# Cyan4973/FiniteStateEntropy

Measured on AMD Instinct MI355X. Metric: MB/s encode+decode per GPU on 32KB probagen blocks; bit-exact vs CPU ref, higher is better.
Workload: dtype u8; 1 GPU; probagen Proba14, 100000 x 32KB blocks per GPU, FSE encode+decode (one-shot calls at the reference's default limits: tableLog 11, decode maxLog 12), bit-exact check; blocks_per_gpu=100000, block_bytes=32768, codec=fse, parity=fse: roundtrip-all-blocks

## Files before the change

finitestateentropy_amd/csrc/fse_tables.hip:

```cpp
#include "internal.h"

#include "wave_glue.h"
#include "ncount_reader.h"
#include "fse_wave_build.h"

template <u32 MAXC>
DEV void fse_wave_build_ctable(const WaveBuildLds& w, const int nn[4], u32 maxSV, u32 tl, u32* img, u32 lane)
{
    u16* const cumAll = w.cumP;
    *(uint2*)(w.nrm + 4 * lane) = make_uint2(((u32)nn[0] & 0xFFFFu) | ((u32)nn[1] << 16), ((u32)nn[2] & 0xFFFFu) | ((u32)nn[3] << 16));
    __syncthreads();
    const u32 ts = 1u << tl;
    u16* const stateTable = (u16*)(img + 1);
    u32* const tt = img + 1 + (ts >> 1);
    {
        u32 eff[4], laneSum = 0;
#pragma unroll
        for (int i = 0; i < 4; ++i) { eff[i] = nn[i] == -1 ? 1u : (u32)nn[i]; laneSum += eff[i]; }
        u32 total;
        u32 run = wb_scan_excl(laneSum, lane, &total);
#pragma unroll
        for (int i = 0; i < 4; ++i) {
            const u32 s = 4 * lane + i;
            cumAll[s] = (u16)run;
            if (s <= maxSV) {
                if (nn[i] == 0) { tt[2 * s] = 0; tt[2 * s + 1] = ((tl + 1) << 16) - ts; }
                else if (nn[i] == -1 || nn[i] == 1) { tt[2 * s] = run - 1u; tt[2 * s + 1] = (tl << 16) - ts; }
                else {
                    const u32 maxBitsOut = tl - hibit32((u32)nn[i] - 1);
                    tt[2 * s] = run - (u32)nn[i];
                    tt[2 * s + 1] = (maxBitsOut << 16) - ((u32)nn[i] << maxBitsOut);
                }
            }
            run += eff[i];
        }
        if (lane == 0) img[0] = tl | (maxSV << 16);
    }
    __syncthreads();
    wave_spread_rank<MAXC>(w, maxSV, tl, lane, [&](u32 s) { return (u32)cumAll[s]; },
                     [&](u32 u, u32 s, u32 r, u32 first) { (void)s; stateTable[first + r] = (u16)(ts + u); });
}

template <u32 MAXC>
__global__ __launch_bounds__(64) void k_fse_cprep(FseCPrepArgs a, u32 capTs)
{
    extern __shared__ __attribute__((aligned(16))) u8 wbLds[];
    const size_t b = blockIdx.x;
    const u32 lane = threadIdx.x;
    const size_t n = view_size(a.src, b);
    FseMeta m; m.state = 0; m.hdrSize = 0; m.tableLog = 0; m.maxSV = 0; m.pace = 0;
    const size_t top = a.histResults[b];
    size_t result = 0; bool go = false;
    if (n <= 1) result = 0;
    else if (is_err(top)) result = top;
    else if (top == n) result = 1;
    else if (top == 1 || top < (n >> 7)) result = 0;
    else go = true;
    const WaveBuildLds w = wave_build_carve(wbLds, capTs, true);
    u32* const hdrImg = w.cnt;
    u32 maxSV = 0, tl = 0;
    int nn[4] = { 0, 0, 0, 0 };
    if (go) {
        maxSV = a.maxSVs[b];
        tl = wg_optimal_tablelog(a.tableLogReq, n, maxSV, 2);
        if ((1u << tl) > 64u * MAXC || (1u << tl) > capTs) { result = FERR(tableLog_tooLarge); go = false; }
    }
    if (go) {
        const uint4 cv = ((const uint4*)(a.counts + b * 256))[lane];
        const u32 c[4] = { cv.x, cv.y, cv.z, cv.w };
        for (u32 i = lane; i < 136; i += 64) hdrImg[i] = 0;
        const size_t e = wg_normalize<64>(nn, c, (u64)n, maxSV, tl, lane);
        if (is_err(e)) { result = e; go = false; }
    }
    __syncthreads();
    if (go) {
        const size_t h = wg_write_ncount<64>(hdrImg, a.dstCapacity, nn, maxSV, tl, lane);
        if (is_err(h)) { result = h; go = false; }
        else m.hdrSize = (u32)h;
    }
    __syncthreads();
    if (!go) { if (lane == 0) { a.meta[b] = m; a.results[b] = result; } return; }
    {   u8* const dst = a.dst + b * a.dstStride;
        const u8* const hb = (const u8*)hdrImg;
        for (u32 i = lane; i < m.hdrSize; i += 64) dst[i] = hb[i];
    }
    int top1 = nn[0] > nn[1] ? nn[0] : nn[1]; top1 = nn[2] > top1 ? nn[2] : top1; top1 = nn[3] > top1 ? nn[3] : top1;
    top1 = wave_max_i32(top1);
    m.state = ((u32)top1 * 64u > (63u << tl) || n < FSE_ENC_WAVE_MIN) ? FSE_ENC_LANE : FSE_ENC_PAR;
    {
        u32 present = (nn[0] != 0) + (nn[1] != 0) + (nn[2] != 0) + (nn[3] != 0);
        present = wg_sum<64>(present);
        const u32 mix = (1u << tl) / (present ? present : 1u);
        m.pace = mix < 64u ? 0u : mix < 128u ? 1u : mix < 256u ? 2u : 3u;
    }
    m.tableLog = tl; m.maxSV = maxSV;
    if (lane == 0) a.meta[b] = m;
    fse_wave_build_ctable<MAXC>(w, nn, maxSV, tl, a.ctables + b * a.ctStrideU32, lane);
}

__global__ __launch_bounds__(64) void k_fse_dparse(FseDPrepArgs a)
{
    __shared__ __attribute__((aligned(16))) u32 stage[NCS_WORDS];
    const size_t b0 = (size_t)blockIdx.x * 64, b = b0 + threadIdx.x;
    const u32 lane = threadIdx.x;
    const bool have = b < a.nBlocks;
    const u8* const in = have ? view_ptr(a.csrc, b) : nullptr;
    const size_t cSize = have ? view_size(a.csrc, b) : 0;
    bool done = false;
    if (have && a.rawRle) { const size_t orig = a.origSizes ? a.origSizes[b] : a.uniformOrig; done = cSize == orig || cSize == 1; }
    const u32 staged = ncount_stage(stage, in, cSize, lane, have && !done);
    {   uint4* const rows = (uint4*)(a.norms + b0 * 256);
        const u32 nRows = a.nBlocks - b0 < 64 ? (u32)(a.nBlocks - b0) : 64u;
        for (u32 i = lane; i < nRows * 32u; i += 64) rows[i] = make_uint4(0, 0, 0, 0);
    }
    __syncthreads();
    int cls = -1;
    if (have) {
        FseMeta m; m.state = 0; m.hdrSize = 0; m.tableLog = 0; m.maxSV = 0; m.pace = 0; m.pace = 0;
        size_t result = 0;
        if (!done) do {
            u32 tl = 0, maxSV = 255;
            s16* const norm = a.norms + b * 256;
            const size_t h = ncount_read_staged(norm, &maxSV, &tl, stage + lane, staged, in, cSize);
            if (is_err(h)) { result = h; break; }
            if (tl > a.maxLog) { result = FERR(tableLog_tooLarge); break; }
            cls = FSE_DCLS_REV11;
            if (tl > FSE_DEC_FAST_MAXLOG) {
                int top = 0;
                for (u32 i = 0; i <= maxSV >> 3; ++i) {
                    const uint4 v = ((const uint4*)norm)[i];
                    const u32 q[4] = { v.x, v.y, v.z, v.w };
#pragma unroll
                    for (int k = 0; k < 4; ++k) { const int lo = (s16)(q[k] & 0xFFFFu), hi = (s16)(q[k] >> 16); top = lo > top ? lo : top; top = hi > top ? hi : top; }
                }
                cls = 2 * top > (1 << tl) ? FSE_DCLS_PLAIN : FSE_DCLS_REV12;
            }
            m.state = 1u | ((u32)cls << 2); m.hdrSize = (u32)h; m.tableLog = tl; m.maxSV = maxSV;
        } while (0);
        a.meta[b] = m;
        if (m.state == 0 && !done) a.results[b] = result;
    }
    if (cls >= 0) { const size_t bin = view_size(a.csrc, b) >> FSE_DBIN_LOG; cls = cls * FSE_DBINS + (int)(bin < FSE_DBINS - 1 ? bin : FSE_DBINS - 1); }
    const unsigned long long below = (1ull << lane) - 1ull;
    unsigned long long todo = __ballot(cls >= 0);
    while (todo) {
        const int leader = __builtin_ctzll(todo);
        const int c = __shfl(cls, leader, WAVE);
        const unsigned long long mask = __ballot(cls == c);
        u32 base = 0;
        if ((int)lane == leader) {
            base = atomicAdd(&a.counts[c], (u32)__builtin_popcountll(mask));
            atomicAdd(&a.counts[FSE_DCLS_COUNT + c / FSE_DBINS], (u32)__builtin_popcountll(mask));
        }
        base = (u32)__shfl((int)base, leader, WAVE);
        if (cls == c) a.lists[(size_t)c * a.nBlocks + base + (u32)__builtin_popcountll(mask & below)] = (u32)b;
        todo &= ~mask;
    }
}

template <u32 MAXC>
__global__ __launch_bounds__(64) void k_fse_dbuild(FseDPrepArgs a, u32 capTs, int firstList, int nLists, u32 ldsCapTs)
{
    extern __shared__ __attribute__((aligned(16))) u8 wbLds[];
    {   u32 total = 0;
        for (int k = firstList / (int)FSE_DBINS; k < (firstList + nLists) / (int)FSE_DBINS; ++k) total += a.counts[FSE_DCLS_COUNT + k];
        if (blockIdx.x >= total) return;
    }
    constexpr int MAXL = 2 * FSE_DBINS;
    static_assert(FSE_DBINS % 4 == 0, "the list lengths are read as 16-byte vectors");
    uint4 cv[MAXL / 4];
#pragma unroll
    for (int i = 0; i < MAXL / 4; ++i) cv[i] = 4 * i < nLists ? ((const uint4*)(a.counts + firstList))[i] : make_uint4(0, 0, 0, 0);
    u32 idx = blockIdx.x;
    int c = firstList + nLists;
    {   u32 before = 0; bool found = false;
#pragma unroll
        for (int i = 0; i < MAXL; ++i) {
            const uint4 v = cv[i >> 2];
            const u32 n = (i & 3) == 0 ? v.x : (i & 3) == 1 ? v.y : (i & 3) == 2 ? v.z : v.w;
            const bool here = !found & (i < nLists) & (idx < before + n);
            c = here ? firstList + i : c; idx = here ? idx - before : idx;
            found |= here;
            before += n;
        }
    }
    if (c == firstList + nLists) return;
    const size_t b = a.lists[(size_t)c * a.nBlocks + idx];
    const u32 lane = threadIdx.x;
    const FseMeta m = a.meta[b];
    if (m.state == 0) return;
    const u32 tl = m.tableLog, ts = 1u << tl;
    if (ts > ldsCapTs || ts > 64u * MAXC) {
        if (lane == 0) { a.meta[b].state = 0; a.results[b] = FERR(tableLog_tooLarge); }
        return;
    }
    const WaveBuildLds w = wave_build_carve(wbLds, ldsCapTs, false);
    *(uint2*)(w.nrm + 4 * lane) = *(const uint2*)(a.norms + b * 256 + 4 * lane);
    __syncthreads();
    const bool rev = ((m.state >> 2) & 3u) != FSE_DCLS_PLAIN;
    u16* const A = a.atab + b * capTs;
    u8* const S = a.symtab + b * capTs;
    const bool fast = wave_spread_rank<MAXC>(w, m.maxSV, tl, lane, [&](u32 s) { return (u32)(int)w.nrm[s]; }, [&](u32 u, u32 s, u32 r, u32 nrm) {
        const int n = (int)nrm;
        const u32 next = (n > 0 ? (u32)n : 1u) + r;
        const u32 nb = tl - hibit32(next);
        const u32 ns = (next << nb) - ts;
        const u32 x = rev ? __brev(u) >> (32u - tl) : u;
        A[x] = rev ? (u16)(nb | ((__brev(ns) >> (32u - tl)) << 5)) : (u16)((ns & 0xFFFu) | (nb << 12));
        S[x] = (u8)s;
    });
    if (lane == 0) a.meta[b].state = m.state | (fast ? 2u : 0u);
}

__global__ __launch_bounds__(256) void k_fse_export_dtable(FseDPrepArgs a, u32 capTs, u32* dtables, size_t dtStrideU32)
{
    const size_t b = blockIdx.x;
    const FseMeta m = a.meta[b];
    if (m.state == 0) return;
    const u32 tl = m.tableLog, ts = 1u << tl;
    const bool rev = ((m.state >> 2) & 3u) != FSE_DCLS_PLAIN;
    const u16* const A = a.atab + b * capTs;
    const u8* const S = a.symtab + b * capTs;
    u32* const dt = dtables + b * dtStrideU32;
    if (threadIdx.x == 0) dt[0] = tl | ((m.state & 2u) ? 1u << 16 : 0u);
    for (u32 x = threadIdx.x; x < ts; x += blockDim.x) {
        const u32 i = rev ? __brev(x) >> (32u - tl) : x;
        const u32 c = A[i];
        const u32 nb = rev ? (c & 31u) : (c >> 12);
        const u32 ns = rev ? __brev(c >> 5) >> (32u - tl) : (c & 0xFFFu);
        dt[1 + x] = ns | ((u32)S[i] << 16) | (nb << 24);
    }
}
hipError_t launch_fse_export_dtables(const FseDPrepArgs& a, u32* dtables, size_t dtStrideU32, hipStream_t s)
{
    if (a.nBlocks == 0) return hipSuccess;
    hipLaunchKernelGGL(k_fse_export_dtable, dim3((unsigned)a.nBlocks), dim3(256), 0, s, a, 1u << a.maxLog, dtables, dtStrideU32);
    return hipGetLastError();
}

DEV size_t fse_norm_load_checked(int nn[4], const s16* nb, u32 maxSV, u32 tl, u32 maxTl, u32 lane)
{
    if (maxSV > 255u) return FERR(maxSymbolValue_tooLarge);
    if (tl > maxTl) return FERR(tableLog_tooLarge);
    if (tl == 0 || tl == 1 || tl == 3) return FERR(GENERIC);
    u32 cells = 0; bool bad = false;
#pragma unroll
    for (int i = 0; i < 4; ++i) {
        nn[i] = 4 * lane + i <= maxSV ? (int)nb[4 * lane + i] : 0;
        bad |= nn[i] < -1;
        cells += nn[i] == -1 ? 1u : nn[i] > 0 ? (u32)nn[i] : 0u;
    }
    cells = wg_sum<64>(cells);
    return (wg_any<64>(bad, lane) || cells != (1u << tl)) ? FERR(GENERIC) : 0;
}
template <u32 MAXC>
__global__ __launch_bounds__(64) void k_fse_ctable_from_norm(const s16* norms, size_t normStride, const u32* maxSVs, u32 tl, u32* ctables, size_t ctStrideU32,
                                                            size_t* results, u32 capTs)
{
    extern __shared__ __attribute__((aligned(16))) u8 wbLds[];
    const size_t b = blockIdx.x;
    const u32 lane = threadIdx.x;
    const u32 maxSV = maxSVs[b];
    int nn[4] = { 0, 0, 0, 0 };
    static_assert(MAXC == 32 || MAXC == 64, "64 * MAXC cells = a table of tableLog 11 or 12");
    const size_t r = fse_norm_load_checked(nn, norms + b * normStride, maxSV, tl, MAXC == 32 ? 11u : FSE_MAX_TL, lane);
    if (lane == 0) results[b] = r;
    if (is_err(r)) return;
    fse_wave_build_ctable<MAXC>(wave_build_carve(wbLds, capTs, true), nn, maxSV, tl, ctables + b * ctStrideU32, lane);
}
hipError_t launch_fse_ctable_from_norm(const s16* norms, size_t normStride, const u32* maxSVs, u32 tl, u32* ctables, size_t ctStrideU32, size_t* results,
                                       size_t nBlocks, hipStream_t s)
{
    if (nBlocks == 0) return hipSuccess;
    const u32 capTs = 1u << (tl >= 1 && tl <= FSE_MAX_TL ? tl : FSE_MAX_TL);
    if (wb_small(capTs))
        hipLaunchKernelGGL(k_fse_ctable_from_norm<32>, dim3((unsigned)nBlocks), dim3(64), wave_build_lds_bytes(capTs, true), s, norms, normStride, maxSVs, tl, ctables,
                           ctStrideU32, results, capTs);
    else
        hipLaunchKernelGGL(k_fse_ctable_from_norm<64>, dim3((unsigned)nBlocks), dim3(64), wave_build_lds_bytes(capTs, true), s, norms, normStride, maxSVs, tl, ctables,
                           ctStrideU32, results, capTs);
    return hipGetLastError();
}

static void launch_fse_dbuild_lists(const FseDPrepArgs& a, u32 capTs, int firstList, int nLists, u32 ldsCapTs, hipStream_t s)
{
    if (wb_small(ldsCapTs))
        hipLaunchKernelGGL(k_fse_dbuild<32>, dim3((unsigned)a.nBlocks), dim3(64), wave_build_lds_bytes(ldsCapTs, false), s, a, capTs, firstList, nLists, ldsCapTs);
    else
        hipLaunchKernelGGL(k_fse_dbuild<64>, dim3((unsigned)a.nBlocks), dim3(64), wave_build_lds_bytes(ldsCapTs, false), s, a, capTs, firstList, nLists, ldsCapTs);
}
static void launch_fse_dbuilds(const FseDPrepArgs& a, hipStream_t s)
{
    const u32 capTs = 1u << a.maxLog;
    const u32 capA = a.maxLog < FSE_DEC_FAST_MAXLOG ? capTs : (1u << FSE_DEC_FAST_MAXLOG);
    launch_fse_dbuild_lists(a, capTs, (int)FSE_DCLS_REV11 * FSE_DBINS, (int)FSE_DBINS, capA, s);
    if (a.maxLog > FSE_DEC_FAST_MAXLOG) launch_fse_dbuild_lists(a, capTs, (int)FSE_DCLS_REV12 * FSE_DBINS, 2 * (int)FSE_DBINS, capTs, s);
}

__global__ __launch_bounds__(64) void k_fse_dmeta_from_norm(FseDPrepArgs a, const s16* norms, size_t normStride, const u32* maxSVs, u32 tl)
{
    const size_t b = blockIdx.x;
    const u32 lane = threadIdx.x;
    const u32 maxSV = maxSVs[b];
    int nn[4] = { 0, 0, 0, 0 };
    const size_t r = fse_norm_load_checked(nn, norms + b * normStride, maxSV, tl, a.maxLog, lane);
    FseMeta m; m.state = 0; m.hdrSize = 0; m.tableLog = tl; m.maxSV = maxSV; m.pace = 0;
    if (!is_err(r)) {
        *(uint2*)(a.norms + b * 256 + 4 * lane) = make_uint2(((u32)nn[0] & 0xFFFFu) | ((u32)nn[1] << 16), ((u32)nn[2] & 0xFFFFu) | ((u32)nn[3] << 16));
        int top = nn[0] > nn[1] ? nn[0] : nn[1]; top = nn[2] > top ? nn[2] : top; top = nn[3] > top ? nn[3] : top;
        top = wave_max_i32(top);
        const u32 cls = tl <= FSE_DEC_FAST_MAXLOG ? (u32)FSE_DCLS_REV11 : 2 * top > (1 << tl) ? (u32)FSE_DCLS_PLAIN : (u32)FSE_DCLS_REV12;
        m.state = 1u | (cls << 2);
        if (lane == 0) {
            const u32 at = atomicAdd(&a.counts[cls * FSE_DBINS], 1u);
            atomicAdd(&a.counts[FSE_DCLS_COUNT + cls], 1u);
            a.lists[(size_t)cls * FSE_DBINS * a.nBlocks + at] = (u32)b;
        }
    }
    if (lane == 0) { a.meta[b] = m; if (is_err(r)) a.results[b] = r; }
}
hipError_t launch_fse_dprep_from_norm(const FseDPrepArgs& a, const s16* norms, size_t normStride, const u32* maxSVs, u32 tl, hipStream_t s)
{
    if (a.nBlocks == 0) return hipSuccess;
    hipError_t e = launch_zero_u32(a.counts, FSE_DCLS_COUNT + FSE_DCLS_KINDS, s);
    if (e != hipSuccess) return e;
    hipLaunchKernelGGL(k_fse_dmeta_from_norm, dim3((unsigned)a.nBlocks), dim3(64), 0, s, a, norms, normStride, maxSVs, tl);
    launch_fse_dbuilds(a, s);
    return hipGetLastError();
}

#ifdef FSE_WB_TIMING
extern "C" __attribute__((visibility("default"))) int FSEHIP_debug_wbTiming(unsigned long long* host) { return (int)hipMemcpyFromSymbol(host, HIP_SYMBOL(g_wbTiming), sizeof(g_wbTiming)); }
#endif
__global__ __launch_bounds__(64) void k_fse_glue_normalize(s16* norms, size_t normStride, u32 tlReq, const u32* counts, size_t countStride,
                                                          const size_t* totals, const u32* maxSVs, size_t* results)
{
    const size_t b = blockIdx.x;
    const u32 lane = threadIdx.x;
    const u32 maxSV = maxSVs[b] > 255u ? 255u : maxSVs[b];
    const u32* const cb = counts + b * countStride;
    u32 c[4];
#pragma unroll
    for (int i = 0; i < 4; ++i) c[i] = 4 * lane + i <= maxSV ? cb[4 * lane + i] : 0u;
    int nn[4] = { 0, 0, 0, 0 };
    const u32 tl = tlReq ? tlReq : FSE_DEF_TL;
    const u64 total = (u64)totals[b];
    size_t r = total ? wg_normalize<64>(nn, c, total, maxSV, tl, lane) : FERR(GENERIC);
    if (!is_err(r)) r = tl;
    s16* const nb = norms + b * normStride;
#pragma unroll
    for (int i = 0; i < 4; ++i) if (4 * lane + i <= maxSV && !is_err(r)) nb[4 * lane + i] = (s16)nn[i];
    if (lane == 0) results[b] = r;
}

__global__ __launch_bounds__(64) void k_fse_glue_write_ncount(u8* headers, size_t headerStride, size_t headerCapacity, const s16* norms, size_t normStride,
                                                             const u32* maxSVs, u32 tl, size_t* results)
{
    __shared__ u32 img[136];
    const size_t b = blockIdx.x;
    const u32 lane = threadIdx.x;
    const u32 maxSV = maxSVs[b];
    size_t r;
    if (tl > FSE_MAX_TL) r = FERR(tableLog_tooLarge);
    else if (tl < FSE_MIN_TL || maxSV > 255u) r = FERR(GENERIC);
    else {
        const s16* const nb = norms + b * normStride;
        int nn[4];
#pragma unroll
        for (int i = 0; i < 4; ++i) nn[i] = 4 * lane + i <= maxSV ? (int)nb[4 * lane + i] : 0;
        for (u32 i = lane; i < 136; i += 64) img[i] = 0;
        __syncthreads();
        r = wg_write_ncount<64>(img, headerCapacity, nn, maxSV, tl, lane);
        __syncthreads();
        if (!is_err(r)) {
            u8* const dst = headers + b * headerStride;
            const u8* const hb = (const u8*)img;
            for (u32 i = lane; i < (u32)r; i += 64) dst[i] = hb[i];
        }
    }
    if (lane == 0) results[b] = r;
}

__global__ __launch_bounds__(64) void k_fse_glue_read_ncount(s16* norms, size_t normStride, u32* maxSVs, u32* tableLogs, BlockView headers, size_t nBlocks, size_t* results)
{
    const size_t b = (size_t)blockIdx.x * 64 + threadIdx.x;
    if (b >= nBlocks) return;
    u32 maxSV = maxSVs[b], tl = 0;
    size_t r;
    if ((size_t)maxSV >= normStride) r = FERR(maxSymbolValue_tooLarge);
    else r = ncount_read<1>(norms + b * normStride, &maxSV, &tl, view_ptr(headers, b), view_size(headers, b));
    if (!is_err(r)) { maxSVs[b] = maxSV; tableLogs[b] = tl; }
    results[b] = r;
}

hipError_t launch_fse_glue_normalize(s16* norms, size_t normStride, u32 tl, const u32* counts, size_t countStride, const size_t* totals, const u32* maxSVs,
                                     size_t* results, size_t nBlocks, hipStream_t s)
{
    if (nBlocks == 0) return hipSuccess;
    hipLaunchKernelGGL(k_fse_glue_normalize, dim3((unsigned)nBlocks), dim3(64), 0, s, norms, normStride, tl, counts, countStride, totals, maxSVs, results);
    return hipGetLastError();
}
hipError_t launch_fse_glue_write_ncount(u8* headers, size_t headerStride, size_t headerCapacity, const s16* norms, size_t normStride, const u32* maxSVs, u32 tl,
                                        size_t* results, size_t nBlocks, hipStream_t s)
{
    if (nBlocks == 0) return hipSuccess;
    hipLaunchKernelGGL(k_fse_glue_write_ncount, dim3((unsigned)nBlocks), dim3(64), 0, s, headers, headerStride, headerCapacity, norms, normStride, maxSVs, tl, results);
    return hipGetLastError();
}
hipError_t launch_fse_glue_read_ncount(s16* norms, size_t normStride, u32* maxSVs, u32* tableLogs, const BlockView& headers, size_t* results, size_t nBlocks, hipStream_t s)
{
    if (nBlocks == 0) return hipSuccess;
    hipLaunchKernelGGL(k_fse_glue_read_ncount, dim3((unsigned)((nBlocks + 63) / 64)), dim3(64), 0, s, norms, normStride, maxSVs, tableLogs, headers, nBlocks, results);
    return hipGetLastError();
}

hipError_t launch_fse_cprep(const FseCPrepArgs& a, hipStream_t s)
{
    if (a.nBlocks == 0) return hipSuccess;
    const u32 capTs = 1u << a.maxTl;
    const size_t ldsBytes = wave_build_lds_bytes(capTs, true);
    probe_before(PK_FSE_CPREP, s);
    if (wb_small(capTs)) hipLaunchKernelGGL(k_fse_cprep<32>, dim3((unsigned)a.nBlocks), dim3(64), ldsBytes, s, a, capTs);
    else hipLaunchKernelGGL(k_fse_cprep<64>, dim3((unsigned)a.nBlocks), dim3(64), ldsBytes, s, a, capTs);
    probe_after(PK_FSE_CPREP, s);
    return hipGetLastError();
}
hipError_t launch_fse_dprep(const FseDPrepArgs& a, hipStream_t s)
{
    if (a.nBlocks == 0) return hipSuccess;
    hipError_t e = launch_zero_u32(a.counts, FSE_DCLS_COUNT + FSE_DCLS_KINDS, s);
    if (e != hipSuccess) return e;
    probe_before(PK_FSE_DPREP, s);
    hipLaunchKernelGGL(k_fse_dparse, dim3((unsigned)((a.nBlocks + 63) / 64)), dim3(64), 0, s, a);
    launch_fse_dbuilds(a, s);
    probe_after(PK_FSE_DPREP, s);
    return hipGetLastError();
}
```

finitestateentropy_amd/csrc/fse_wave_build.h:

```cpp
#pragma once
#include "dev_common.h"

#define WB_MAXSYM 256
#ifndef WB_WIN
#define WB_WIN 64u
#endif
#define WB_TSTEP(ts) (((ts) >> 1) + ((ts) >> 3) + 3)

#ifdef FSE_WB_TIMING
__device__ unsigned long long g_wbTiming[4096 * 8];
#define WBT(k) TT[k] = __builtin_readcyclecounter();
#else
#define WBT(k)
#endif
struct WaveBuildLds {
    s16* nrm;
    u16* cumP;
    u8*  symP;
    u8*  symTab;
    u8*  marks;
    u32* cnt;
    u16* coarse;
};
__host__ __device__ inline u32 wb_si(u32 u) { return u + ((u >> 5) << 2); }
#ifndef WB_EXTRA_LDS
#define WB_EXTRA_LDS 0u
#endif
__host__ __device__ inline size_t wb_up16(size_t n) { return (n + 15) & ~(size_t)15; }
__host__ __device__ inline size_t wb_part_a(u32 capTs) { const size_t m = wb_si(capTs); return wb_up16(m > WB_WIN * 64 ? m : WB_WIN * 64); }
__host__ __device__ inline size_t wb_part_b(u32 capTs) { const size_t t = wb_si(capTs); return wb_up16(t > WB_WIN * 32 ? t : WB_WIN * 32); }
__host__ __device__ inline size_t wave_build_lds_bytes(u32 capTs, bool withCum) { return wb_part_a(capTs) + wb_part_b(capTs) + 512 + 256 + (withCum ? 528 : 0) + WB_EXTRA_LDS; }
DEV WaveBuildLds wave_build_carve(u8* base, u32 capTs, bool withCum)
{
    WaveBuildLds w;
    w.cnt = (u32*)base; w.marks = base; base += wb_part_a(capTs);
    w.coarse = (u16*)base; w.symTab = base; base += wb_part_b(capTs);
    w.nrm = (s16*)base; base += 512;
    w.symP = base; base += 256;
    w.cumP = withCum ? (u16*)base : nullptr;
    return w;
}
__host__ __device__ inline bool wb_small(u32 capTs) { return capTs <= 2048u; }

DEV u32 wb_bytesum(u32 v) { return __builtin_amdgcn_sad_u8(v, 0u, 0u); }
DEV u32 wb_scan_excl(u32 v, u32 lane, u32* total)
{
#if FSEHIP_DPP_SCANS
    const u32 incl = group_scan_incl<64, ScanAdd>(v, lane);
    *total = group_last<64>(incl, lane);
#else
    u32 incl = v;
#pragma unroll
    for (int off = 1; off < 64; off <<= 1) { const u32 o = (u32)__shfl_up((int)incl, off, WAVE); if ((int)lane >= off) incl += o; }
    *total = (u32)__shfl((int)incl, 63, WAVE);
#endif
    return incl - v;
}

DEV void wb_opaque(u32& v) { asm volatile("" : "+v"(v)); }
#define WB_MAXC ((1u << FSEHIP_FSE_MAX_TABLELOG) >> 6)

template <u32 MAXC, class Payload, class Emit>
DEV bool wave_spread_rank(const WaveBuildLds& w, u32 maxSV, u32 tl, u32 lane, Payload&& payload, Emit&& emit)
{
#ifdef FSE_WB_TIMING
    unsigned long long TT[8];
#endif
    WBT(0)
    const u32 ts = 1u << tl, mask = ts - 1, step = WB_TSTEP(ts);
    const u32 C = ts >= 64 ? ts >> 6 : 1;
    const bool act = lane * C < ts;
    const u32 m0 = lane * C;
    static_assert(MAXC % 8 == 0 && MAXC <= WB_MAXC, "cells per lane: whole groups of eight, at most the largest table's");
    u8* const marks = w.marks;
    int n[4];
    {   const uint2 raw = *(const uint2*)(w.nrm + 4 * lane);
        n[0] = (s16)(raw.x & 0xFFFFu); n[1] = (s16)(raw.x >> 16); n[2] = (s16)(raw.y & 0xFFFFu); n[3] = (s16)(raw.y >> 16);
    }
    u32 lanePos = 0, laneLow = 0, laneAny = 0; bool big = false;
#pragma unroll
    for (int i = 0; i < 4; ++i) {
        if (4 * lane + i > maxSV) n[i] = 0;
        lanePos += n[i] > 0 ? (u32)n[i] : 0u; laneLow += n[i] == -1; laneAny += n[i] != 0;
        big |= n[i] >= (int)(ts >> 1);
    }
    u32 totals;
    const u32 base3 = wb_scan_excl(lanePos | (laneLow << 13) | (laneAny << 22), lane, &totals);
    u32 posBase = base3 & 0x1FFFu, lowBase = (base3 >> 13) & 0x1FFu, anyBase = base3 >> 22;
    const u32 nLow = (totals >> 13) & 0x1FFu, nAny = totals >> 22;
    const int high = (int)ts - 1 - (int)nLow;
    if (act) { if (C >= 4) for (u32 i = 0; i < C; i += 4) *(u32*)(marks + wb_si(m0 + i)) = 0; else for (u32 i = 0; i < C; ++i) marks[wb_si(m0 + i)] = 0; }
    __syncthreads();
    WBT(1)
#pragma unroll
    for (int i = 0; i < 4; ++i) {
        if (n[i] != 0) w.symP[anyBase++] = (u8)(4 * lane + i);
        if (n[i] > 0) { marks[wb_si(posBase)] = (u8)(4 * lane + i); posBase += (u32)n[i]; }
        else if (n[i] == -1) { w.symTab[wb_si(ts - 1 - lowBase)] = (u8)(4 * lane + i); ++lowBase; }
    }
    u32 nv = 0;
    if (act) { u32 u = (m0 * step) & mask; for (u32 i = 0; i < C; ++i) { nv += (int)u <= high; u = (u + step) & mask; } }
    u32 totalKept;
    const u32 k0 = wb_scan_excl(nv, lane, &totalKept);
    __syncthreads();
    WBT(2)
    u32 localMax = 0;
    for (u32 i = 0; i < nv; i += 8) {
        u32 v[8];
#pragma unroll
        for (u32 j = 0; j < 8; ++j) { const u32 idx = k0 + i + j; v[j] = marks[wb_si(idx < ts ? idx : ts - 1)]; }
#pragma unroll
        for (u32 j = 0; j < 8; ++j) if (i + j < nv) localMax = v[j] > localMax ? v[j] : localMax;
    }
    u32 run = localMax;
#if FSEHIP_DPP_SCANS
    run = group_scan_incl<64, ScanMax>(run, lane);
    run = dpp_mov<0x138, 0xF, true>(0u, run);
#else
#pragma unroll
    for (int off = 1; off < 64; off <<= 1) { const u32 o = (u32)__shfl_up((int)run, off, WAVE); if ((int)lane >= off) run = o > run ? o : run; }
    run = (u32)__shfl_up((int)run, 1, WAVE);
    if (lane == 0) run = 0;
#endif
    if (act && nv) {
        u32 u = (m0 * step) & mask, k = k0;
        u32 i = 0;
        for (; i + 8 <= C; i += 8) {
            u32 uu[8], v[8]; bool keep[8];
#pragma unroll
            for (u32 j = 0; j < 8; ++j) {
                uu[j] = u; keep[j] = (int)u <= high;
                v[j] = marks[wb_si(k < ts ? k : ts - 1)];
                k += keep[j]; u = (u + step) & mask;
            }
#pragma unroll
            for (u32 j = 0; j < 8; ++j) if (keep[j]) { run = v[j] > run ? v[j] : run; w.symTab[wb_si(uu[j])] = (u8)run; }
        }
        for (; i < C; ++i) {
            if ((int)u <= high) { const u32 v = marks[wb_si(k)]; ++k; run = v > run ? v : run; w.symTab[wb_si(u)] = (u8)run; }
            u = (u + step) & mask;
        }
    }
    __syncthreads();
    WBT(3)

    const u32 nj = C < 8 ? C : 8;
    u32 sym[MAXC / 4], lr[MAXC / 4];
#pragma unroll
    for (u32 q = 0; q < MAXC / 4; ++q) { sym[q] = 0; lr[q] = 0; }
    if (act) {
        if (C >= 8) {
#pragma unroll
            for (u32 g = 0; g < MAXC / 8; ++g)
                if (8 * g < C) {
                    const u32* const syp = (const u32*)(w.symTab + wb_si(m0 + 8 * g));
                    sym[2 * g] = syp[0]; sym[2 * g + 1] = syp[1];
                }
        } else {
#pragma unroll
            for (u32 j = 0; j < 4; ++j) if (j < C) sym[0] |= (u32)w.symTab[wb_si(m0 + j)] << (8 * j);
        }
    }
    const u32 sh8 = 8 * (lane & 3u), grp = lane >> 2;
    const u32 belowMask = (1u << sh8) - 1u;
    const bool single = maxSV < WB_WIN;
    for (u32 base = 0; base <= maxSV; base += WB_WIN) {
        {   const u32 rows = (maxSV + 1 - base) < WB_WIN ? (maxSV + 1 - base) : WB_WIN;
            for (u32 i = 4 * lane; i < rows * 16; i += 256) *(uint4*)(w.cnt + i) = make_uint4(0, 0, 0, 0);
        }
        __syncthreads();
        if (act) {
#pragma unroll
            for (u32 g = 0; g < MAXC / 8; ++g) {
                if (8 * g >= C) break;
                wb_opaque(sym[2 * g]); wb_opaque(sym[2 * g + 1]);
                u32 old[8]; bool in[8];
#pragma unroll
                for (u32 j = 0; j < 8; ++j) {
                    const u32 s = ((sym[2 * g + (j >> 2)] >> (8 * (j & 3))) & 0xFFu) - base;
                    in[j] = j < nj && (single || s < WB_WIN);
                    old[j] = 0;
                    if (in[j]) old[j] = atomicAdd(&w.cnt[s * 16 + grp], 1u << sh8);
                }
#pragma unroll
                for (u32 h = 0; h < 2; ++h) {
                    u32 r = lr[2 * g + h];
#pragma unroll
                    for (u32 k = 0; k < 4; ++k) {
                        const u32 j = 4 * h + k;
                        if (in[j]) r = (r & ~(0xFFu << (8 * k))) | (((old[j] >> sh8) & 0xFFu) << (8 * k));
                    }
                    lr[2 * g + h] = r;
                }
            }
        }
        __syncthreads();
        WBT(4)
        for (u32 j = lane; j < nAny; j += 64) {
            const u32 s = (u32)w.symP[j] - base;
            if (!single && s >= WB_WIN) continue;
            const uint4* const row = (const uint4*)(w.cnt + s * 16);
            const uint4 c0 = row[0], c1 = row[1], c2 = row[2], c3 = row[3];
            u32 r[16];
            u32 acc = 0;
#define WB_ACC(k, v) r[k] = acc; acc += wb_bytesum(v);
            WB_ACC(0, c0.x) WB_ACC(1, c0.y) WB_ACC(2, c0.z) WB_ACC(3, c0.w) WB_ACC(4, c1.x) WB_ACC(5, c1.y) WB_ACC(6, c1.z) WB_ACC(7, c1.w)
            WB_ACC(8, c2.x) WB_ACC(9, c2.y) WB_ACC(10, c2.z) WB_ACC(11, c2.w) WB_ACC(12, c3.x) WB_ACC(13, c3.y) WB_ACC(14, c3.z) WB_ACC(15, c3.w)
#undef WB_ACC
            uint4* const out = (uint4*)(w.coarse + s * 16);
            out[0] = make_uint4(r[0] | (r[1] << 16), r[2] | (r[3] << 16), r[4] | (r[5] << 16), r[6] | (r[7] << 16));
            out[1] = make_uint4(r[8] | (r[9] << 16), r[10] | (r[11] << 16), r[12] | (r[13] << 16), r[14] | (r[15] << 16));
        }
        __syncthreads();
        WBT(5)
        if (act) {
#pragma unroll
            for (u32 g = 0; g < MAXC / 8; ++g) {
                if (8 * g >= C) break;
                wb_opaque(sym[2 * g]); wb_opaque(sym[2 * g + 1]);
                u32 mg = m0 + 8 * g; wb_opaque(mg);
                u32 sf[8], co[8], cn[8], pl[8]; bool in[8];
#pragma unroll
                for (u32 j = 0; j < 8; ++j) {
                    sf[j] = (sym[2 * g + (j >> 2)] >> (8 * (j & 3))) & 0xFFu;
                    const u32 sw = sf[j] - base;
                    in[j] = j < nj && (single || sw < WB_WIN);
                    const u32 row = in[j] ? sw : 0u;
                    co[j] = w.coarse[row * 16 + grp]; cn[j] = w.cnt[row * 16 + grp]; pl[j] = payload(sf[j]);
                }
#pragma unroll
                for (u32 j = 0; j < 8; ++j) {
                    const u32 local = (lr[2 * g + (j >> 2)] >> (8 * (j & 3))) & 0xFFu;
                    if (in[j]) emit(mg + j, sf[j], local + co[j] + wb_bytesum(cn[j] & belowMask), pl[j]);
                }
            }
        }
        __syncthreads();
    }
    WBT(6)
#ifdef FSE_WB_TIMING
    if (lane == 0 && blockIdx.x < 4096) for (int q = 0; q < 6; ++q) g_wbTiming[8 * blockIdx.x + q] = TT[q + 1] - TT[q];
#endif
    return !__any(big);
}
```

Baseline: 207,900 MiB/s of uncompressed data through encode+decode (whole job).

## Persist dbuild<64> blocks over list entries and fold payload into coarse prefix

For large tables, the decode-table build kernel now launches a capped grid (a fixed number of blocks per CU) and each block loops over its list entries, using readfirstlane to keep the block id and metadata scalar. The spread/rank helper now adds the per-symbol payload into the coarse prefix once per symbol, instead of fetching it per element, and the emit callback takes one combined slot value. An extra opaque barrier on lr is meant to curb register pressure in the 64-wide variant. The aim is to cut per-element work and launch/occupancy overhead for 4K tables. The risks are less parallelism when many blocks need building and added loop overhead, and the coarse prefix may overflow its 16-bit packing.

```diff
diff --git a/finitestateentropy_amd/csrc/fse_tables.hip b/finitestateentropy_amd/csrc/fse_tables.hip
--- a/finitestateentropy_amd/csrc/fse_tables.hip
+++ b/finitestateentropy_amd/csrc/fse_tables.hip
@@ -38,7 +38,7 @@
     }
     __syncthreads();
     wave_spread_rank<MAXC>(w, maxSV, tl, lane, [&](u32 s) { return (u32)cumAll[s]; },
-                     [&](u32 u, u32 s, u32 r, u32 first) { (void)s; stateTable[first + r] = (u16)(ts + u); });
+                     [&](u32 u, u32 s, u32 slot) { (void)s; stateTable[slot] = (u16)(ts + u); });
 }
 
 template <u32 MAXC>
@@ -162,54 +162,57 @@
 __global__ __launch_bounds__(64) void k_fse_dbuild(FseDPrepArgs a, u32 capTs, int firstList, int nLists, u32 ldsCapTs)
 {
     extern __shared__ __attribute__((aligned(16))) u8 wbLds[];
-    {   u32 total = 0;
-        for (int k = firstList / (int)FSE_DBINS; k < (firstList + nLists) / (int)FSE_DBINS; ++k) total += a.counts[FSE_DCLS_COUNT + k];
-        if (blockIdx.x >= total) return;
-    }
+    u32 total = 0;
+    for (int k = firstList / (int)FSE_DBINS; k < (firstList + nLists) / (int)FSE_DBINS; ++k) total += a.counts[FSE_DCLS_COUNT + k];
+    if (blockIdx.x >= total) return;
     constexpr int MAXL = 2 * FSE_DBINS;
     static_assert(FSE_DBINS % 4 == 0, "the list lengths are read as 16-byte vectors");
     uint4 cv[MAXL / 4];
 #pragma unroll
     for (int i = 0; i < MAXL / 4; ++i) cv[i] = 4 * i < nLists ? ((const uint4*)(a.counts + firstList))[i] : make_uint4(0, 0, 0, 0);
-    u32 idx = blockIdx.x;
-    int c = firstList + nLists;
-    {   u32 before = 0; bool found = false;
-#pragma unroll
-        for (int i = 0; i < MAXL; ++i) {
-            const uint4 v = cv[i >> 2];
-            const u32 n = (i & 3) == 0 ? v.x : (i & 3) == 1 ? v.y : (i & 3) == 2 ? v.z : v.w;
-            const bool here = !found & (i < nLists) & (idx < before + n);
-            c = here ? firstList + i : c; idx = here ? idx - before : idx;
-            found |= here;
-            before += n;
-        }
-    }
-    if (c == firstList + nLists) return;
-    const size_t b = a.lists[(size_t)c * a.nBlocks + idx];
-    const u32 lane = threadIdx.x;
-    const FseMeta m = a.meta[b];
-    if (m.state == 0) return;
-    const u32 tl = m.tableLog, ts = 1u << tl;
-    if (ts > ldsCapTs || ts > 64u * MAXC) {
-        if (lane == 0) { a.meta[b].state = 0; a.results[b] = FERR(tableLog_tooLarge); }
-        return;
-    }
     const WaveBuildLds w = wave_build_carve(wbLds, ldsCapTs, false);
-    *(uint2*)(w.nrm + 4 * lane) = *(const uint2*)(a.norms + b * 256 + 4 * lane);
-    __syncthreads();
-    const bool rev = ((m.state >> 2) & 3u) != FSE_DCLS_PLAIN;
-    u16* const A = a.atab + b * capTs;
-    u8* const S = a.symtab + b * capTs;
-    const bool fast = wave_spread_rank<MAXC>(w, m.maxSV, tl, lane, [&](u32 s) { return (u32)(int)w.nrm[s]; }, [&](u32 u, u32 s, u32 r, u32 nrm) {
-        const int n = (int)nrm;
-        const u32 next = (n > 0 ? (u32)n : 1u) + r;
-        const u32 nb = tl - hibit32(next);
-        const u32 ns = (next << nb) - ts;
-        const u32 x = rev ? __brev(u) >> (32u - tl) : u;
-        A[x] = rev ? (u16)(nb | ((__brev(ns) >> (32u - tl)) << 5)) : (u16)((ns & 0xFFFu) | (nb << 12));
-        S[x] = (u8)s;
-    });
-    if (lane == 0) a.meta[b].state = m.state | (fast ? 2u : 0u);
+    for (u32 at = blockIdx.x; at < total; at += gridDim.x) {
+        u32 lane = threadIdx.x; wb_opaque(lane);
+        u32 idx = at;
+        int c = firstList + nLists;
+        {   u32 before = 0; bool found = false;
+#pragma unroll
+            for (int i = 0; i < MAXL; ++i) {
+                const uint4 v = cv[i >> 2];
+                const u32 n = (i & 3) == 0 ? v.x : (i & 3) == 1 ? v.y : (i & 3) == 2 ? v.z : v.w;
+                const bool here = !found & (i < nLists) & (idx < before + n);
+                c = here ? firstList + i : c; idx = here ? idx - before : idx;
+                found |= here;
+                before += n;
+            }
+        }
+        if (c == firstList + nLists) return;
+        const size_t b = (u32)__builtin_amdgcn_readfirstlane((int)a.lists[(size_t)c * a.nBlocks + idx]);
+        FseMeta m = a.meta[b];
+        m.state = (u32)__builtin_amdgcn_readfirstlane((int)m.state); m.tableLog = (u32)__builtin_amdgcn_readfirstlane((int)m.tableLog);
+        m.maxSV = (u32)__builtin_amdgcn_readfirstlane((int)m.maxSV);
+        if (m.state == 0) continue;
+        const u32 tl = m.tableLog, ts = 1u << tl;
+        if (ts > ldsCapTs || ts > 64u * MAXC) {
+            if (lane == 0) { a.meta[b].state = 0; a.results[b] = FERR(tableLog_tooLarge); }
+            continue;
+        }
+        *(uint2*)(w.nrm + 4 * lane) = *(const uint2*)(a.norms + b * 256 + 4 * lane);
+        __syncthreads();
+        const bool rev = ((m.state >> 2) & 3u) != FSE_DCLS_PLAIN;
+        u16* const A = a.atab + b * capTs;
+        u8* const S = a.symtab + b * capTs;
+        const bool fast = wave_spread_rank<MAXC>(w, m.maxSV, tl, lane, [&](u32 s) { const int n = (int)w.nrm[s]; return n > 0 ? (u32)n : 1u; },
+                                                [&](u32 u, u32 s, u32 next) {
+            const u32 nb = tl - hibit32(next);
+            const u32 ns = (next << nb) - ts;
+            const u32 x = rev ? __brev(u) >> (32u - tl) : u;
+            A[x] = rev ? (u16)(nb | ((__brev(ns) >> (32u - tl)) << 5)) : (u16)((ns & 0xFFFu) | (nb << 12));
+            S[x] = (u8)s;
+        });
+        if (lane == 0) a.meta[b].state = m.state | (fast ? 2u : 0u);
+        if (MAXC == 32) break;
+    }
 }
 
 __global__ __launch_bounds__(256) void k_fse_export_dtable(FseDPrepArgs a, u32 capTs, u32* dtables, size_t dtStrideU32)
@@ -282,12 +285,16 @@
     return hipGetLastError();
 }
 
+#define FSE_DBUILD12_PER_CU 16
 static void launch_fse_dbuild_lists(const FseDPrepArgs& a, u32 capTs, int firstList, int nLists, u32 ldsCapTs, hipStream_t s)
 {
     if (wb_small(ldsCapTs))
         hipLaunchKernelGGL(k_fse_dbuild<32>, dim3((unsigned)a.nBlocks), dim3(64), wave_build_lds_bytes(ldsCapTs, false), s, a, capTs, firstList, nLists, ldsCapTs);
-    else
-        hipLaunchKernelGGL(k_fse_dbuild<64>, dim3((unsigned)a.nBlocks), dim3(64), wave_build_lds_bytes(ldsCapTs, false), s, a, capTs, firstList, nLists, ldsCapTs);
+    else {
+        const size_t cap = (size_t)FSE_DBUILD12_PER_CU * (size_t)(dev_props().ok ? dev_props().cus : 256);
+        hipLaunchKernelGGL(k_fse_dbuild<64>, dim3((unsigned)(a.nBlocks < cap ? a.nBlocks : cap)), dim3(64), wave_build_lds_bytes(ldsCapTs, false), s, a, capTs, firstList,
+                           nLists, ldsCapTs);
+    }
 }
 static void launch_fse_dbuilds(const FseDPrepArgs& a, hipStream_t s)
 {
diff --git a/finitestateentropy_amd/csrc/fse_wave_build.h b/finitestateentropy_amd/csrc/fse_wave_build.h
--- a/finitestateentropy_amd/csrc/fse_wave_build.h
+++ b/finitestateentropy_amd/csrc/fse_wave_build.h
@@ -174,6 +174,7 @@
             for (u32 g = 0; g < MAXC / 8; ++g) {
                 if (8 * g >= C) break;
                 wb_opaque(sym[2 * g]); wb_opaque(sym[2 * g + 1]);
+                if (MAXC > 32 && g) wb_opaque(lr[2 * g - 1]);
                 u32 old[8]; bool in[8];
 #pragma unroll
                 for (u32 j = 0; j < 8; ++j) {
@@ -199,10 +200,11 @@
         for (u32 j = lane; j < nAny; j += 64) {
             const u32 s = (u32)w.symP[j] - base;
             if (!single && s >= WB_WIN) continue;
+            const u32 pay = payload(s + base);
             const uint4* const row = (const uint4*)(w.cnt + s * 16);
             const uint4 c0 = row[0], c1 = row[1], c2 = row[2], c3 = row[3];
             u32 r[16];
-            u32 acc = 0;
+            u32 acc = pay;
 #define WB_ACC(k, v) r[k] = acc; acc += wb_bytesum(v);
             WB_ACC(0, c0.x) WB_ACC(1, c0.y) WB_ACC(2, c0.z) WB_ACC(3, c0.w) WB_ACC(4, c1.x) WB_ACC(5, c1.y) WB_ACC(6, c1.z) WB_ACC(7, c1.w)
             WB_ACC(8, c2.x) WB_ACC(9, c2.y) WB_ACC(10, c2.z) WB_ACC(11, c2.w) WB_ACC(12, c3.x) WB_ACC(13, c3.y) WB_ACC(14, c3.z) WB_ACC(15, c3.w)
@@ -219,19 +221,19 @@
                 if (8 * g >= C) break;
                 wb_opaque(sym[2 * g]); wb_opaque(sym[2 * g + 1]);
                 u32 mg = m0 + 8 * g; wb_opaque(mg);
-                u32 sf[8], co[8], cn[8], pl[8]; bool in[8];
+                u32 sf[8], co[8], cn[8]; bool in[8];
 #pragma unroll
                 for (u32 j = 0; j < 8; ++j) {
                     sf[j] = (sym[2 * g + (j >> 2)] >> (8 * (j & 3))) & 0xFFu;
                     const u32 sw = sf[j] - base;
                     in[j] = j < nj && (single || sw < WB_WIN);
                     const u32 row = in[j] ? sw : 0u;
-                    co[j] = w.coarse[row * 16 + grp]; cn[j] = w.cnt[row * 16 + grp]; pl[j] = payload(sf[j]);
+                    co[j] = w.coarse[row * 16 + grp]; cn[j] = w.cnt[row * 16 + grp];
                 }
 #pragma unroll
                 for (u32 j = 0; j < 8; ++j) {
                     const u32 local = (lr[2 * g + (j >> 2)] >> (8 * (j & 3))) & 0xFFu;
-                    if (in[j]) emit(mg + j, sf[j], local + co[j] + wb_bytesum(cn[j] & belowMask), pl[j]);
+                    if (in[j]) emit(mg + j, sf[j], local + co[j] + wb_bytesum(cn[j] & belowMask));
                 }
             }
         }
```

After: 207,300 MiB/s of uncompressed data through encode+decode (whole job). No clear change (-0.3%).

## Add branch-free fast path for wave table build and ballot-based list lookup

Applied to the files above, without the earlier changes.

Adds a specialised fast path in the wave spread/rank builder for the common case: a single symbol window with at least eight cells per lane. It skips the per-element bounds predicates and uses perm/ubfe to pack ranks, and replaces predicated LDS stores with stores to a dummy slot. It also skips the low-probability counting loop when there are no -1 symbols. In the decode-table build kernel, the serial unrolled scan over list counts is replaced by a wave-wide scan plus ballot, and the reversed/plain selection becomes mask-select arithmetic. This adds code size and register pressure through the extra template path, and relies on dummy LDS slots that must not collide with live data.

```diff
diff --git a/finitestateentropy_amd/csrc/fse_tables.hip b/finitestateentropy_amd/csrc/fse_tables.hip
--- a/finitestateentropy_amd/csrc/fse_tables.hip
+++ b/finitestateentropy_amd/csrc/fse_tables.hip
@@ -167,26 +167,22 @@
         if (blockIdx.x >= total) return;
     }
     constexpr int MAXL = 2 * FSE_DBINS;
-    static_assert(FSE_DBINS % 4 == 0, "the list lengths are read as 16-byte vectors");
-    uint4 cv[MAXL / 4];
-#pragma unroll
-    for (int i = 0; i < MAXL / 4; ++i) cv[i] = 4 * i < nLists ? ((const uint4*)(a.counts + firstList))[i] : make_uint4(0, 0, 0, 0);
+    static_assert(MAXL <= 64, "one lane per list");
+    const u32 lane = threadIdx.x;
     u32 idx = blockIdx.x;
     int c = firstList + nLists;
-    {   u32 before = 0; bool found = false;
-#pragma unroll
-        for (int i = 0; i < MAXL; ++i) {
-            const uint4 v = cv[i >> 2];
-            const u32 n = (i & 3) == 0 ? v.x : (i & 3) == 1 ? v.y : (i & 3) == 2 ? v.z : v.w;
-            const bool here = !found & (i < nLists) & (idx < before + n);
-            c = here ? firstList + i : c; idx = here ? idx - before : idx;
-            found |= here;
-            before += n;
+    {   const u32 n = (int)lane < nLists ? a.counts[firstList + (int)lane] : 0u;
+        u32 all;
+        const u32 before = wb_scan_excl(n, lane, &all);
+        const unsigned long long hit = __ballot(idx >= before && idx - before < n);
+        if (hit) {
+            const int l = __builtin_ctzll(hit);
+            c = firstList + l;
+            idx -= (u32)__builtin_amdgcn_readlane((int)before, l);
         }
     }
     if (c == firstList + nLists) return;
     const size_t b = a.lists[(size_t)c * a.nBlocks + idx];
-    const u32 lane = threadIdx.x;
     const FseMeta m = a.meta[b];
     if (m.state == 0) return;
     const u32 tl = m.tableLog, ts = 1u << tl;
@@ -200,13 +196,17 @@
     const bool rev = ((m.state >> 2) & 3u) != FSE_DCLS_PLAIN;
     u16* const A = a.atab + b * capTs;
     u8* const S = a.symtab + b * capTs;
+    u32 revMask = rev ? ~0u : 0u;
+    wb_opaque(revMask);
+    const u32 shr = 32u - tl;
     const bool fast = wave_spread_rank<MAXC>(w, m.maxSV, tl, lane, [&](u32 s) { return (u32)(int)w.nrm[s]; }, [&](u32 u, u32 s, u32 r, u32 nrm) {
         const int n = (int)nrm;
         const u32 next = (n > 0 ? (u32)n : 1u) + r;
         const u32 nb = tl - hibit32(next);
         const u32 ns = (next << nb) - ts;
-        const u32 x = rev ? __brev(u) >> (32u - tl) : u;
-        A[x] = rev ? (u16)(nb | ((__brev(ns) >> (32u - tl)) << 5)) : (u16)((ns & 0xFFFu) | (nb << 12));
+        const u32 x = wb_pick(revMask, __brev(u) >> shr, u);
+        const u32 cell = wb_pick(revMask, nb | ((__brev(ns) >> shr) << 5), (ns & 0xFFFu) | (nb << 12));
+        *(u16*)((u8*)A + (x << 1)) = (u16)cell;
         S[x] = (u8)s;
     });
     if (lane == 0) a.meta[b].state = m.state | (fast ? 2u : 0u);
diff --git a/finitestateentropy_amd/csrc/fse_wave_build.h b/finitestateentropy_amd/csrc/fse_wave_build.h
--- a/finitestateentropy_amd/csrc/fse_wave_build.h
+++ b/finitestateentropy_amd/csrc/fse_wave_build.h
@@ -1,12 +1,20 @@
 #pragma once
 #include "dev_common.h"
+#include <type_traits>
 
 #define WB_MAXSYM 256
 #ifndef WB_WIN
 #define WB_WIN 64u
 #endif
 #define WB_TSTEP(ts) (((ts) >> 1) + ((ts) >> 3) + 3)
-
+#define WB_DUMMY 32u
+
+#ifndef WB_PATHS
+#define WB_PATHS 3
+#endif
+#ifndef WB_FAST_MAXC
+#define WB_FAST_MAXC 32u
+#endif
 #ifdef FSE_WB_TIMING
 __device__ unsigned long long g_wbTiming[4096 * 8];
 #define WBT(k) TT[k] = __builtin_readcyclecounter();
@@ -43,6 +51,7 @@
 __host__ __device__ inline bool wb_small(u32 capTs) { return capTs <= 2048u; }
 
 DEV u32 wb_bytesum(u32 v) { return __builtin_amdgcn_sad_u8(v, 0u, 0u); }
+DEV u32 wb_pick(u32 mask, u32 a, u32 b) { return (a & mask) | (b & ~mask); }
 DEV u32 wb_scan_excl(u32 v, u32 lane, u32* total)
 {
 #if FSEHIP_DPP_SCANS
@@ -94,23 +103,28 @@
     WBT(1)
 #pragma unroll
     for (int i = 0; i < 4; ++i) {
-        if (n[i] != 0) w.symP[anyBase++] = (u8)(4 * lane + i);
-        if (n[i] > 0) { marks[wb_si(posBase)] = (u8)(4 * lane + i); posBase += (u32)n[i]; }
-        else if (n[i] == -1) { w.symTab[wb_si(ts - 1 - lowBase)] = (u8)(4 * lane + i); ++lowBase; }
-    }
-    u32 nv = 0;
-    if (act) { u32 u = (m0 * step) & mask; for (u32 i = 0; i < C; ++i) { nv += (int)u <= high; u = (u + step) & mask; } }
+        const u32 s = 4 * lane + i;
+        const bool any = n[i] != 0, pos = n[i] > 0, low = n[i] == -1;
+        w.symP[any ? anyBase : 255u] = (u8)s;
+        marks[pos ? wb_si(posBase) : WB_DUMMY] = (u8)s;
+        w.symTab[low ? wb_si(ts - 1 - lowBase) : WB_DUMMY] = (u8)s;
+        anyBase += any; posBase += pos ? (u32)n[i] : 0u; lowBase += low;
+    }
+    u32 nv = act ? C : 0u;
+    if (nLow != 0 && act) { u32 u = (m0 * step) & mask; nv = 0; for (u32 i = 0; i < C; ++i) { nv += (int)u <= high; u = (u + step) & mask; } }
     u32 totalKept;
     const u32 k0 = wb_scan_excl(nv, lane, &totalKept);
     __syncthreads();
     WBT(2)
     u32 localMax = 0;
-    for (u32 i = 0; i < nv; i += 8) {
-        u32 v[8];
-#pragma unroll
-        for (u32 j = 0; j < 8; ++j) { const u32 idx = k0 + i + j; v[j] = marks[wb_si(idx < ts ? idx : ts - 1)]; }
-#pragma unroll
-        for (u32 j = 0; j < 8; ++j) if (i + j < nv) localMax = v[j] > localMax ? v[j] : localMax;
+    {   const u32 kLast = k0 + nv - 1;
+        for (u32 i = 0; i < nv; i += 8) {
+            u32 v[8];
+#pragma unroll
+            for (u32 j = 0; j < 8; ++j) { const u32 idx = k0 + i + j; v[j] = marks[wb_si(idx < kLast ? idx : kLast)]; }
+#pragma unroll
+            for (u32 j = 0; j < 8; ++j) localMax = v[j] > localMax ? v[j] : localMax;
+        }
     }
     u32 run = localMax;
 #if FSEHIP_DPP_SCANS
@@ -126,15 +140,16 @@
         u32 u = (m0 * step) & mask, k = k0;
         u32 i = 0;
         for (; i + 8 <= C; i += 8) {
-            u32 uu[8], v[8]; bool keep[8];
+            u32 at[8], v[8];
 #pragma unroll
             for (u32 j = 0; j < 8; ++j) {
-                uu[j] = u; keep[j] = (int)u <= high;
+                const bool keep = (int)u <= high;
+                at[j] = keep ? wb_si(u) : WB_DUMMY;
                 v[j] = marks[wb_si(k < ts ? k : ts - 1)];
-                k += keep[j]; u = (u + step) & mask;
-            }
-#pragma unroll
-            for (u32 j = 0; j < 8; ++j) if (keep[j]) { run = v[j] > run ? v[j] : run; w.symTab[wb_si(uu[j])] = (u8)run; }
+                k += keep; u = (u + step) & mask;
+            }
+#pragma unroll
+            for (u32 j = 0; j < 8; ++j) { run = v[j] > run ? v[j] : run; w.symTab[at[j]] = (u8)run; }
         }
         for (; i < C; ++i) {
             if ((int)u <= high) { const u32 v = marks[wb_si(k)]; ++k; run = v > run ? v : run; w.symTab[wb_si(u)] = (u8)run; }
@@ -146,8 +161,6 @@
 
     const u32 nj = C < 8 ? C : 8;
     u32 sym[MAXC / 4], lr[MAXC / 4];
-#pragma unroll
-    for (u32 q = 0; q < MAXC / 4; ++q) { sym[q] = 0; lr[q] = 0; }
     if (act) {
         if (C >= 8) {
 #pragma unroll
@@ -157,38 +170,52 @@
                     sym[2 * g] = syp[0]; sym[2 * g + 1] = syp[1];
                 }
         } else {
+            sym[0] = 0; sym[1] = 0;
 #pragma unroll
             for (u32 j = 0; j < 4; ++j) if (j < C) sym[0] |= (u32)w.symTab[wb_si(m0 + j)] << (8 * j);
         }
     }
-    const u32 sh8 = 8 * (lane & 3u), grp = lane >> 2;
-    const u32 belowMask = (1u << sh8) - 1u;
     const bool single = maxSV < WB_WIN;
-    for (u32 base = 0; base <= maxSV; base += WB_WIN) {
+    auto window = [&](auto fastTag, const u32 base) {
+        constexpr bool FAST = decltype(fastTag)::value;
+        u32 ln = lane; wb_opaque(ln);
+        const u32 sh8 = 8 * (ln & 3u), grp = ln >> 2;
+        const u32 belowMask = (1u << sh8) - 1u, inc = 1u << sh8;
         {   const u32 rows = (maxSV + 1 - base) < WB_WIN ? (maxSV + 1 - base) : WB_WIN;
             for (u32 i = 4 * lane; i < rows * 16; i += 256) *(uint4*)(w.cnt + i) = make_uint4(0, 0, 0, 0);
         }
         __syncthreads();
-        if (act) {
+        if (FAST) {
+            const u32 selLo = 0x0C0C0000u | (ln & 3u) | ((4u + (ln & 3u)) << 8), selHi = 0x00000C0Cu | (selLo << 16);
 #pragma unroll
             for (u32 g = 0; g < MAXC / 8; ++g) {
                 if (8 * g >= C) break;
                 wb_opaque(sym[2 * g]); wb_opaque(sym[2 * g + 1]);
-                u32 old[8]; bool in[8];
+                u32 old[8];
+#pragma unroll
+                for (u32 j = 0; j < 8; ++j) old[j] = atomicAdd(&w.cnt[__builtin_amdgcn_ubfe(sym[2 * g + (j >> 2)], 8 * (j & 3), 8u) * 16 + grp], inc);
+                lr[2 * g] = __builtin_amdgcn_perm(old[1], old[0], selLo) | __builtin_amdgcn_perm(old[3], old[2], selHi);
+                lr[2 * g + 1] = __builtin_amdgcn_perm(old[5], old[4], selLo) | __builtin_amdgcn_perm(old[7], old[6], selHi);
+            }
+        } else if (act) {
+#pragma unroll
+            for (u32 g = 0; g < MAXC / 8; ++g) {
+                if (8 * g >= C) break;
+                wb_opaque(sym[2 * g]); wb_opaque(sym[2 * g + 1]);
+                u32 old[8];
 #pragma unroll
                 for (u32 j = 0; j < 8; ++j) {
                     const u32 s = ((sym[2 * g + (j >> 2)] >> (8 * (j & 3))) & 0xFFu) - base;
-                    in[j] = j < nj && (single || s < WB_WIN);
-                    old[j] = 0;
-                    if (in[j]) old[j] = atomicAdd(&w.cnt[s * 16 + grp], 1u << sh8);
+                    old[j] = ~0u;
+                    if (j < nj && (single || s < WB_WIN)) old[j] = atomicAdd(&w.cnt[s * 16 + grp], inc);
                 }
 #pragma unroll
                 for (u32 h = 0; h < 2; ++h) {
                     u32 r = lr[2 * g + h];
 #pragma unroll
                     for (u32 k = 0; k < 4; ++k) {
-                        const u32 j = 4 * h + k;
-                        if (in[j]) r = (r & ~(0xFFu << (8 * k))) | (((old[j] >> sh8) & 0xFFu) << (8 * k));
+                        const u32 o = old[4 * h + k], put = (r & ~(0xFFu << (8 * k))) | (((o >> sh8) & 0xFFu) << (8 * k));
+                        r = o != ~0u ? put : r;
                     }
                     lr[2 * g + h] = r;
                 }
@@ -198,7 +225,7 @@
         WBT(4)
         for (u32 j = lane; j < nAny; j += 64) {
             const u32 s = (u32)w.symP[j] - base;
-            if (!single && s >= WB_WIN) continue;
+            if (!FAST && !single && s >= WB_WIN) continue;
             const uint4* const row = (const uint4*)(w.cnt + s * 16);
             const uint4 c0 = row[0], c1 = row[1], c2 = row[2], c3 = row[3];
             u32 r[16];
@@ -213,30 +240,58 @@
         }
         __syncthreads();
         WBT(5)
-        if (act) {
+        if (FAST) {
 #pragma unroll
             for (u32 g = 0; g < MAXC / 8; ++g) {
                 if (8 * g >= C) break;
                 wb_opaque(sym[2 * g]); wb_opaque(sym[2 * g + 1]);
-                u32 mg = m0 + 8 * g; wb_opaque(mg);
-                u32 sf[8], co[8], cn[8], pl[8]; bool in[8];
+                u32 mg = m0; wb_opaque(mg); mg += 8 * g;
+                u32 sf[8], co[8], cn[8], pl[8];
+#pragma unroll
+                for (u32 j = 0; j < 8; ++j) {
+                    sf[j] = __builtin_amdgcn_ubfe(sym[2 * g + (j >> 2)], 8 * (j & 3), 8u);
+                    co[j] = w.coarse[sf[j] * 16 + grp]; cn[j] = w.cnt[sf[j] * 16 + grp]; pl[j] = payload(sf[j]);
+                }
+#pragma unroll
+                for (u32 j = 0; j < 8; ++j)
+                    emit(mg + j, sf[j], __builtin_amdgcn_ubfe(lr[2 * g + (j >> 2)], 8 * (j & 3), 8u) + co[j] + wb_bytesum(cn[j] & belowMask), pl[j]);
+            }
+        } else if (act) {
+#pragma unroll
+            for (u32 g = 0; g < MAXC / 8; ++g) {
+                if (8 * g >= C) break;
+                wb_opaque(sym[2 * g]); wb_opaque(sym[2 * g + 1]);
+                u32 mg = m0; wb_opaque(mg); mg += 8 * g;
+                u32 sf[8], co[8], cn[8], pl[8];
 #pragma unroll
                 for (u32 j = 0; j < 8; ++j) {
                     sf[j] = (sym[2 * g + (j >> 2)] >> (8 * (j & 3))) & 0xFFu;
                     const u32 sw = sf[j] - base;
-                    in[j] = j < nj && (single || sw < WB_WIN);
-                    const u32 row = in[j] ? sw : 0u;
+                    const u32 row = (j < nj && (single || sw < WB_WIN)) ? sw : 0u;
                     co[j] = w.coarse[row * 16 + grp]; cn[j] = w.cnt[row * 16 + grp]; pl[j] = payload(sf[j]);
                 }
 #pragma unroll
                 for (u32 j = 0; j < 8; ++j) {
                     const u32 local = (lr[2 * g + (j >> 2)] >> (8 * (j & 3))) & 0xFFu;
-                    if (in[j]) emit(mg + j, sf[j], local + co[j] + wb_bytesum(cn[j] & belowMask), pl[j]);
+                    if (j < nj && (single || sf[j] - base < WB_WIN)) emit(mg + j, sf[j], local + co[j] + wb_bytesum(cn[j] & belowMask), pl[j]);
                 }
             }
         }
         __syncthreads();
-    }
+    };
+#if WB_PATHS & 1
+    if (WB_FAST_MAXC >= MAXC && single && C >= 8) window(std::true_type{}, 0u);
+    else
+#endif
+#if WB_PATHS & 2
+    {
+#pragma unroll
+        for (u32 q = 0; q < MAXC / 4; ++q) lr[q] = 0;
+        for (u32 base = 0; base <= maxSV; base += WB_WIN) window(std::false_type{}, base);
+    }
+#else
+    {}
+#endif
     WBT(6)
 #ifdef FSE_WB_TIMING
     if (lane == 0 && blockIdx.x < 4096) for (int q = 0; q < 6; ++q) g_wbTiming[8 * blockIdx.x + q] = TT[q + 1] - TT[q];
```

Result: no change. 206,800 MiB/s of uncompressed data through encode+decode (whole job) before, 208,800 MiB/s of uncompressed data through encode+decode (whole job) after, median of 6 (+0.9%).
